# deepreinforce-ai/CUDA-L2

Measured on AMD Instinct MI355X. Metric: HGEMM TFLOP/s, higher is better.
Workload: dtype f16

## Files before the change

### cuda-l2_amd/build.py

```python
from __future__ import annotations

import concurrent.futures as cf
import hashlib
import os
import shutil
import subprocess
import sys
from pathlib import Path

PKG_DIR = Path(__file__).resolve().parent
REPO_DIR = PKG_DIR.parent
CSRC = PKG_DIR / "csrc"
INCLUDE = REPO_DIR / "include"
BUILD = PKG_DIR / "build"
OBJ = BUILD / "obj"
_SUFFIX = os.environ.get("HGEMM_LIB_SUFFIX", "")
LIB_DIR = PKG_DIR / ("lib_" + _SUFFIX if _SUFFIX else "lib")
BIN_DIR = PKG_DIR / "bin"
ROCM = Path(os.environ.get("ROCM_PATH", "/opt/rocm"))
HIPCC = str(ROCM / "bin" / "hipcc")
ARCH = "gfx950"

LIB_SOURCES = [
    "hgemm_inst_g0.hip",
    "hgemm_inst_g1.hip",
    "hgemm_inst_g2.hip",
    "hgemm_inst_g3.hip",
    "hgemm_inst_g4.hip",
    "hgemm_inst_g5.hip",
    "hgemm_inst_g6.hip",
    "hgemm_inst_g7.hip",
    "hgemm_inst_g8.hip",
    "hgemm_inst_g9.hip",
    "hgemm_inst_g10.hip",
    "hgemm_inst_g11.hip",
    "hgemm_inst_g12.hip",
    "hgemm_registry.hip",
    "hgemm_plan.hip",
    "hgemm_api.hip",
    "hgemm_baselines.hip",
]

HIP_FLAGS = os.environ.get("HGEMM_EXTRA_HIPFLAGS", "").split() + [f"--offload-arch={ARCH}", "-O3", "-std=c++17", "-fPIC", "-Wall", "-Wno-unused-function",
             "-Wno-unused-result", "-Wno-unused-value", "-DROCBLAS_NO_DEPRECATED_WARNINGS", "-D__HIP_PLATFORM_AMD__"]


def _headers_digest() -> str:
    h = hashlib.sha256()
    for d in (CSRC, INCLUDE):
        for p in sorted(d.rglob("*")):
            if p.suffix in (".hpp", ".h", ".def", ".inc"):
                h.update(p.name.encode())
                h.update(p.read_bytes())
    return h.hexdigest()


def _run(cmd: list[str], verbose: bool) -> None:
    if verbose:
        print(" ".join(cmd), flush=True)
    res = subprocess.run(cmd, capture_output=True, text=True)
    if res.returncode != 0:
        sys.stderr.write(res.stdout + res.stderr)
        raise RuntimeError(f"build step failed ({res.returncode}): {' '.join(cmd)}")
    if verbose and (res.stdout or res.stderr):
        print(res.stdout + res.stderr, flush=True)


def compile_object(src: Path, extra_flags: list[str], hdr_digest: str, verbose: bool = False) -> Path:
    OBJ.mkdir(parents=True, exist_ok=True)
    cmd_core = [HIPCC, *HIP_FLAGS, *extra_flags, f"-I{CSRC}", f"-I{INCLUDE}", "-c"]
    key = hashlib.sha256()
    key.update(" ".join(cmd_core).encode())
    key.update(hdr_digest.encode())
    key.update(src.read_bytes())
    obj = OBJ / f"{src.stem}-{key.hexdigest()[:20]}.o"
    if not obj.exists():
        tmp = obj.with_suffix(f".tmp{os.getpid()}.o")
        _run([*cmd_core, str(src), "-o", str(tmp)], verbose)
        os.replace(tmp, obj)
    return obj


def build_library(verbose: bool = False, jobs: int | None = None) -> Path:
    hdr = _headers_digest()
    jobs = jobs or min(8, os.cpu_count() or 1)
    srcs = [CSRC / s for s in LIB_SOURCES]
    with cf.ThreadPoolExecutor(max_workers=jobs) as ex:
        objs = list(ex.map(lambda s: compile_object(s, [], hdr, verbose), srcs))
    LIB_DIR.mkdir(exist_ok=True)
    lib = LIB_DIR / "libhgemm_mi355x.so"
    stamp = LIB_DIR / ".libhgemm_mi355x.stamp"
    want = hashlib.sha256(" ".join(o.name for o in objs).encode()).hexdigest()
    if lib.exists() and stamp.exists() and stamp.read_text() == want:
        return lib
    tmp = lib.with_suffix(f".tmp{os.getpid()}.so")
    _run([HIPCC, f"--offload-arch={ARCH}", "-shared", "-fPIC", *map(str, objs), "-o", str(tmp),
          f"-L{ROCM / 'lib'}", "-lrocblas", "-lhipblaslt", "-lamdhip64",
          "-Wl,--no-undefined", "-Wl,-soname,libhgemm_mi355x.so"], verbose)
    os.replace(tmp, lib)
    stamp.write_text(want)
    return lib


def build_tools(verbose: bool = False) -> list[Path]:
    lib = build_library(verbose)
    hdr = _headers_digest()
    BIN_DIR.mkdir(exist_ok=True)
    out = []
    for name in ("hgemm_tune",):
        src = CSRC / "tools" / f"{name}.cpp"
        if not src.exists():
            continue
        obj = compile_object(src, ["-x", "hip"], hdr, verbose)
        exe = BIN_DIR / name
        stamp = BIN_DIR / f".{name}.stamp"
        want = obj.name + lib.name + str(lib.stat().st_mtime_ns)
        if not (exe.exists() and stamp.exists() and stamp.read_text() == want):
            _run([HIPCC, f"--offload-arch={ARCH}", str(obj), "-o", str(exe), f"-L{LIB_DIR}", "-lhgemm_mi355x",
                  f"-L{ROCM / 'lib'}", "-lamdhip64", "-lrocm_smi64", "-Wl,-rpath,$ORIGIN/../lib", f"-Wl,-rpath,{ROCM / 'lib'}"],
# ... 61 lines not shown
```

### cuda-l2_amd/csrc/hgemm_api.hip

```cpp
#include "hgemm_plan.hpp"
#include "hgemm_kernel_nn.hpp"
#include "../../include/hgemm_mi355x.h"

#include <algorithm>
#include <atomic>
#include <cmath>
#include <cstdint>
#include <cstdlib>
#include <cstring>
#include <mutex>
#include <vector>

using namespace hgemm_mi355x;

namespace {

thread_local int g_last_hip_error = 0;
#ifdef HGEMM_ABLATION
int g_debug_flags = 0;
#endif
#ifdef HGEMM_TIMELINE
unsigned long long* g_timeline = nullptr;
int g_timeline_slots = 0;
unsigned g_timeline_count = 0;
// ... 664 lines not shown
  for (Workspace& w : g_ws)
    if (w.ptr && hipFree(w.ptr) != hipSuccess) rc = HGEMM_ERR_HIP;
  for (void* p : g_ws_retired)
    if (hipFree(p) != hipSuccess) rc = HGEMM_ERR_HIP;
  g_ws.clear();
  g_ws_retired.clear();
  return rc;
}

int hgemm_mi355x_release_stream_workspace(void* stream) {
  int dev = 0;
  if (hipGetDevice(&dev) != hipSuccess) return HGEMM_ERR_HIP;
  std::lock_guard<std::mutex> lk(g_ws_mutex);
  for (size_t i = 0; i < g_ws.size(); ++i) {
    if (g_ws[i].device != dev || g_ws[i].stream != (hipStream_t)stream) continue;
    int rc = HGEMM_OK;
    if (g_ws[i].ptr) {
      if (g_ws[i].captured) g_ws_retired.push_back(g_ws[i].ptr);
      else if (hipFree(g_ws[i].ptr) != hipSuccess) rc = HGEMM_ERR_HIP;
    }
    g_ws.erase(g_ws.begin() + (long)i);
    return rc;
  }
  return HGEMM_OK;
}

int hgemm_mi355x_reserve_workspace(int M, int N, int K, void* stream) {
  if (M <= 0 || N <= 0 || K <= 0) return HGEMM_ERR_BAD_ARG;
  int cfg = 0, splits = 1, group = 1;
  const int st = hgemm_mi355x_plan(M, N, K, &cfg, &splits, &group);
  if (st != HGEMM_OK) return st;
  const size_t ws = std::max(hgemm_mi355x_plan_workspace_bytes(cfg, splits, M, N, K), kCounterBytes + (size_t)256 * 256 * 256 * sizeof(float));
  float* slabs = nullptr; unsigned* counters = nullptr;
  const int rc = ensure_workspace(ws - kCounterBytes, (hipStream_t)stream, &slabs, &counters);
  return rc == HGEMM_ERR_NO_WORKSPACE_INTERNAL ? HGEMM_ERR_NO_WORKSPACE : rc;
}

int hgemm_mi355x_launch(int config_id, int splits_arg, int group_m, const void* a, const void* b,
                        const void* b_col_major, void* c, int M, int N, int K, int lda, int ldb,
                        int ldc, void* stream) {
  DisarmTiming disarm_timing;
  if (!a || !c || M <= 0 || N <= 0 || K <= 0) return HGEMM_ERR_BAD_ARG;
  if (config_id >= g_num_kernels || config_id < HGEMM_CONFIG_RAGGED) return HGEMM_ERR_BAD_ARG;
#ifdef HGEMM_TIMELINE
  ++g_timeline_count;
#endif
  hipStream_t s = (hipStream_t)stream;
  const bool aligned = mfma_path_ok(a, b_col_major, c, M, N, K, lda, ldb, ldc);
  unsigned ruled_out = 0;
  auto resolve = [&] {
    return resolve_launch(config_id, splits_arg, group_m, b != nullptr, b_col_major != nullptr, aligned, M, N, K, lda, ldb, ldc, ruled_out);
  };
  LaunchPlan p = resolve();
  float* slabs = nullptr; unsigned* counters = nullptr;
  while (p.status == HGEMM_OK && p.slab_bytes) {
    const int st = ensure_workspace(p.slab_bytes, s, &slabs, &counters);
    if (st == HGEMM_OK) break;
    if (st != HGEMM_ERR_NO_WORKSPACE_INTERNAL && p.form != FORM_HYBRID) return st;
    ruled_out |= 1u << p.form;
    p = resolve();
  }
  if (p.status != HGEMM_OK) return p.status;
  for (int i = 0; i < p.n; ++i) {
    GemmArgs& g = p.d[i].g;
    g.A = (const f16*)a; g.Bt = (const f16*)b_col_major; g.C = (f16*)c;
    if (p.d[i].epi != EPI_C16) {
      g.partial = slabs;
      if (p.counters) g.counters = counters;
    }
    const TimingSlot ts = timing_slot(p.d[i].start, p.d[i].stop);
    switch (p.d[i].thunk) {
      case THUNK_ENTRY: g_kernel_table[config_id].launch(g, p.d[i].grid, s, p.d[i].epi, ts); break;
      case THUNK_SPLITK_REDUCE: launch_splitk_reduce(g.partial, g.C, M, N, ldc, g.splits, s, ts); break;
      case THUNK_TAIL_REDUCE: launch_tail_reduce(g, g_kernel_table[config_id].bm, g_kernel_table[config_id].bn, s, ts); break;
      case THUNK_RAGGED: launch_ragged(g, s, ts); break;
      case THUNK_GENERIC: launch_generic((const f16*)a, (const f16*)b, (f16*)c, M, N, K, lda, N, ldc, s, ts); break;
    }
  }
  hipError_t err = hipGetLastError();
  if (err != hipSuccess) { g_last_hip_error = (int)err; return HGEMM_ERR_HIP; }
  return HGEMM_OK;
}

int hgemm_mi355x_set_insitu(int enable) {
  const int old = insitu_enabled() ? 1 : 0;
  g_insitu_mode.store(enable ? 1 : 0);
  if (!enable) {
    std::lock_guard<std::mutex> lk(g_insitu_mutex);
    g_insitu.clear();
    g_insitu_epoch.fetch_add(1, std::memory_order_release);
  }
  return old;
}

int hgemm_mi355x_insitu_enabled(void) { return insitu_enabled() ? 1 : 0; }

int hgemm_mi355x_insitu_candidates(int M, int N, int K, int config_id[3], int splits[3], int group_m[3]) {
  if (M <= 0 || N <= 0 || K <= 0 || !config_id || !splits || !group_m) return 0;
  PlanTriple c[3];
  const int n = insitu_candidates(M, N, K, c);
  for (int i = 0; i < n; ++i) { config_id[i] = c[i].cfg; splits[i] = c[i].splits; group_m[i] = c[i].group_m; }
  return n;
}

int hgemm_mi355x_insitu_choice(int M, int N, int K, int* config_id, int* splits, int* group_m) {
  PlanTriple p;
  int dev = 0;
  if (hipGetDevice(&dev) != hipSuccess) { (void)hipGetLastError(); dev = 0; }
  if (!config_id || !splits || !group_m || !insitu_lookup(dev, M, N, K, &p)) return 0;
  *config_id = p.cfg; *splits = p.splits; *group_m = p.group_m;
  return 1;
}

int hgemm_mi355x_fp32(const void* a, const void* b, const void* bt, void* c, int M, int N, int K,
                      void* stream) {
  return run(HGEMM_ACC_FP32, a, b, bt, c, M, N, K, stream);
}

int hgemm_mi355x_fp16(const void* a, const void* b, const void* bt, void* c, int M, int N, int K,
                      void* stream) {
  return run(HGEMM_ACC_FP16, a, b, bt, c, M, N, K, stream);
}

int hgemm_mi355x_nn_num_configs(void) { return kLayoutNN.t.count; }
const char* hgemm_mi355x_nn_config_name(int id) { return tr_config_name(kLayoutNN, id); }
int hgemm_mi355x_nn_config_by_name(const char* name) { return tr_config_by_name(kLayoutNN, name); }
int hgemm_mi355x_nn_config_info(int id, int out[8]) { return tr_config_info(kLayoutNN, id, out); }
int hgemm_mi355x_nn_plan(int M, int N, int K, int* nn_config, int* splits) { return tr_plan(kLayoutNN, M, N, K, nn_config, splits); }
int hgemm_mi355x_nn_runs(int nn_config, int M, int N, int K, int lda, int ldb, int ldc) { return tr_runs(kLayoutNN, TR_F16, kOutC16, nn_config, M, N, K, lda, ldb, ldc); }
size_t hgemm_mi355x_nn_plan_workspace_bytes(int nn_config, int splits, int M, int N, int K) {
  return tr_plan_workspace_bytes(kLayoutNN, nn_config, splits, M, N, K);
}
int hgemm_mi355x_nn_reserve_workspace(int M, int N, int K, void* stream) { return tr_reserve_workspace(kLayoutNN, M, N, K, stream); }
int hgemm_mi355x_launch_nn(int nn_config, int splits_arg, const void* a, const void* b, void* c, int M, int N, int K, int lda, int ldb,
                           int ldc, void* stream) {
  return tr_launch(kLayoutNN, TR_F16, kOutC16, nn_config, splits_arg, a, b, nullptr, c, M, N, K, lda, ldb, ldc, stream);
}
int hgemm_mi355x_nn_fp32(const void* a, const void* b, void* c, int M, int N, int K, void* stream) { return tr_run(kLayoutNN, TR_F16, kOutC16, a, b, nullptr, c, M, N, K, stream); }
int hgemm_mi355x_nn_fp16(const void* a, const void* b, void* c, int M, int N, int K, void* stream) { return tr_run(kLayoutNN, TR_F16, kOutC16, a, b, nullptr, c, M, N, K, stream); }
int hgemm_mi355x_selfcheck_launch_nn(int nn_config, int splits, int operands, int M, int N, int K, int lda, int ldb, int ldc, int ruled_out,
                                     long long out[20]) {
  return tr_selfcheck_launch(kLayoutNN, TR_F16, kOutC16, nn_config, splits, operands, M, N, K, lda, ldb, ldc, ruled_out, out);
}

int hgemm_mi355x_ta_num_configs(void) { return kLayoutTA.t.count; }
const char* hgemm_mi355x_ta_config_name(int id) { return tr_config_name(kLayoutTA, id); }
int hgemm_mi355x_ta_config_by_name(const char* name) { return tr_config_by_name(kLayoutTA, name); }
int hgemm_mi355x_ta_config_info(int id, int out[8]) { return tr_config_info(kLayoutTA, id, out); }
int hgemm_mi355x_ta_plan(int M, int N, int K, int* ta_config, int* splits) { return tr_plan(kLayoutTA, M, N, K, ta_config, splits); }
int hgemm_mi355x_ta_runs(int ta_config, int M, int N, int K, int lda, int ldb, int ldc) { return tr_runs(kLayoutTA, TR_F16, kOutC16, ta_config, M, N, K, lda, ldb, ldc); }
size_t hgemm_mi355x_ta_plan_workspace_bytes(int ta_config, int splits, int M, int N, int K) {
  return tr_plan_workspace_bytes(kLayoutTA, ta_config, splits, M, N, K);
}
int hgemm_mi355x_ta_reserve_workspace(int M, int N, int K, void* stream) { return tr_reserve_workspace(kLayoutTA, M, N, K, stream); }
int hgemm_mi355x_launch_ta(int ta_config, int splits_arg, const void* a_col_major, const void* b, void* c, int M, int N, int K, int lda,
                           int ldb, int ldc, void* stream) {
  return tr_launch(kLayoutTA, TR_F16, kOutC16, ta_config, splits_arg, a_col_major, b, nullptr, c, M, N, K, lda, ldb, ldc, stream);
}
int hgemm_mi355x_ta_fp32(const void* a_col_major, const void* b, void* c, int M, int N, int K, void* stream) { return tr_run(kLayoutTA, TR_F16, kOutC16, a_col_major, b, nullptr, c, M, N, K, stream); }
int hgemm_mi355x_ta_fp16(const void* a_col_major, const void* b, void* c, int M, int N, int K, void* stream) { return tr_run(kLayoutTA, TR_F16, kOutC16, a_col_major, b, nullptr, c, M, N, K, stream); }
int hgemm_mi355x_selfcheck_launch_ta(int ta_config, int splits, int operands, int M, int N, int K, int lda, int ldb, int ldc, int ruled_out,
                                     long long out[20]) {
  return tr_selfcheck_launch(kLayoutTA, TR_F16, kOutC16, ta_config, splits, operands, M, N, K, lda, ldb, ldc, ruled_out, out);
}

int hgemm_mi355x_launch_ta_c32(int ta_config, int splits_arg, const void* a_col_major, const void* b, float* c32, int M, int N, int K, int lda,
// ... 180 lines not shown
```

### cuda-l2_amd/csrc/hgemm_launch.hpp

```cpp
#pragma once
#include "hgemm_kernel_rs.hpp"
#include "hgemm_kernel_sq.hpp"
#include "hgemm_kernel_wd.hpp"
#include "hgemm_kernel_lu.hpp"

#include <hip/hip_ext.h>

namespace hgemm_mi355x {

struct LaunchTiming { hipEvent_t start = nullptr, stop = nullptr; };
extern thread_local LaunchTiming t_launch_timing;

struct TimingSlot { hipEvent_t start = nullptr, stop = nullptr; };
inline TimingSlot timing_slot(bool first, bool last) {
  TimingSlot s;
  if (first) { s.start = t_launch_timing.start; t_launch_timing.start = nullptr; }
  if (last) { s.stop = t_launch_timing.stop; t_launch_timing.stop = nullptr; }
  return s;
}

#define HGEMM_LAUNCH(KERNEL, GRID, THREADS, STREAM, SLOT, ...)                                              \
  do {                                                                                                      \
    if ((SLOT).start || (SLOT).stop)                                                                        \
      hipExtLaunchKernelGGL(KERNEL, dim3(GRID), dim3(THREADS), 0, STREAM, (SLOT).start, (SLOT).stop, 0,     \
                            __VA_ARGS__);                                                                   \
    else                                                                                                    \
      hipLaunchKernelGGL(KERNEL, dim3(GRID), dim3(THREADS), 0, STREAM, __VA_ARGS__);                        \
  } while (0)

template <class CFG>
void launch_cfg(const GemmArgs& g, int grid, hipStream_t stream, int epi, TimingSlot ts) {
  if (epi == EPI_STREAMK) {
    if constexpr (CFG::BM * CFG::BN <= 256 * 128) HGEMM_LAUNCH((hgemm_tn_sk_kernel<CFG>), grid, CFG::THREADS, stream, ts, g);
  } else if (epi == EPI_FUSED)
    HGEMM_LAUNCH((hgemm_tn_kernel<CFG, EPI_FUSED>), grid, CFG::THREADS, stream, ts, g);
  else if (epi == EPI_SLAB)
    HGEMM_LAUNCH((hgemm_tn_kernel<CFG, EPI_SLAB>), grid, CFG::THREADS, stream, ts, g);
  else
    HGEMM_LAUNCH((hgemm_tn_kernel<CFG, EPI_C16>), grid, CFG::THREADS, stream, ts, g);
}

template <class CFG>
void launch_sp(const GemmArgs& g, int grid, hipStream_t stream, int epi, TimingSlot ts) {
  const bool wide = ((g.N & 7) == 0) && ((g.ldc & 7) == 0) && ((reinterpret_cast<uintptr_t>(g.C) & 15) == 0);
  if (epi == EPI_FUSED)
    HGEMM_LAUNCH((hgemm_tn_sp_kernel<CFG, SP_EPI_FUSED>), grid, CFG::THREADS, stream, ts, g);
  else if (epi == EPI_SLAB)
    HGEMM_LAUNCH((hgemm_tn_sp_kernel<CFG, SP_EPI_SLAB>), grid, CFG::THREADS, stream, ts, g);
  else if (wide)
    HGEMM_LAUNCH((hgemm_tn_sp_kernel<CFG, SP_EPI_WIDE>), grid, CFG::THREADS, stream, ts, g);
  else
    HGEMM_LAUNCH((hgemm_tn_sp_kernel<CFG, SP_EPI_NARROW>), grid, CFG::THREADS, stream, ts, g);
}

template <class CFG, int FLAG>
void launch_sq_variant(const GemmArgs& g, int grid, hipStream_t stream, int epi, TimingSlot ts) {
  const bool wide = ((g.N & 7) == 0) && ((g.ldc & 7) == 0) && ((reinterpret_cast<uintptr_t>(g.C) & 15) == 0);
  if (epi == EPI_FUSED)
    HGEMM_LAUNCH((hgemm_tn_sq_kernel<CFG, SP_EPI_FUSED | FLAG>), grid, CFG::THREADS, stream, ts, g);
  else if (epi == EPI_SLAB)
    HGEMM_LAUNCH((hgemm_tn_sq_kernel<CFG, SP_EPI_SLAB | FLAG>), grid, CFG::THREADS, stream, ts, g);
  else if (wide)
    HGEMM_LAUNCH((hgemm_tn_sq_kernel<CFG, SP_EPI_WIDE | FLAG>), grid, CFG::THREADS, stream, ts, g);
  else
    HGEMM_LAUNCH((hgemm_tn_sq_kernel<CFG, SP_EPI_NARROW | FLAG>), grid, CFG::THREADS, stream, ts, g);
}

template <class CFG>
void launch_sq(const GemmArgs& g, int grid, hipStream_t stream, int epi, TimingSlot ts) {
  if constexpr (CFG::MI == 16) {
    if (g.K % (BK * CFG::KT) != 0) return launch_sq_variant<CFG, EPI_KTAIL>(g, grid, stream, epi, ts);
    if (g.flags & ARG_XCD_STAGGER) return launch_sq_variant<CFG, EPI_KSTAGGER>(g, grid, stream, epi, ts);
  }
  launch_sq_variant<CFG, 0>(g, grid, stream, epi, ts);
}

template <class CFG, int FLAG>
void launch_rs_variant(const GemmArgs& g, int grid, hipStream_t stream, int epi, TimingSlot ts) {
  if (epi == EPI_FUSED)
    HGEMM_LAUNCH((hgemm_tn_rs_kernel<CFG, EPI_FUSED | FLAG>), grid, CFG::THREADS, stream, ts, g);
  else if (epi == EPI_SLAB)
    HGEMM_LAUNCH((hgemm_tn_rs_kernel<CFG, EPI_SLAB | FLAG>), grid, CFG::THREADS, stream, ts, g);
  else
    HGEMM_LAUNCH((hgemm_tn_rs_kernel<CFG, EPI_C16 | FLAG>), grid, CFG::THREADS, stream, ts, g);
}

template <class CFG>
void launch_rs(const GemmArgs& g, int grid, hipStream_t stream, int epi, TimingSlot ts) {
  if (epi == EPI_STREAMK)
    HGEMM_LAUNCH((hgemm_tn_rs_sk_kernel<CFG>), grid, CFG::THREADS, stream, ts, g);
  else if (g.K % CFG::BKS != 0)
    launch_rs_variant<CFG, EPI_KTAIL>(g, grid, stream, epi, ts);
  else
    launch_rs_variant<CFG, 0>(g, grid, stream, epi, ts);
}

template <class CFG>
void launch_wd(const GemmArgs& g, int grid, hipStream_t stream, int epi, TimingSlot ts) {
  if (epi == EPI_FUSED)
    HGEMM_LAUNCH((hgemm_tn_wd_kernel<CFG, EPI_FUSED>), grid, CFG::THREADS, stream, ts, g);
  else if (epi == EPI_SLAB)
    HGEMM_LAUNCH((hgemm_tn_wd_kernel<CFG, EPI_SLAB>), grid, CFG::THREADS, stream, ts, g);
  else
    HGEMM_LAUNCH((hgemm_tn_wd_kernel<CFG, EPI_C16>), grid, CFG::THREADS, stream, ts, g);
}

template <class CFG>
void launch_lu(const GemmArgs& g, int grid, hipStream_t stream, int epi, TimingSlot ts) {
  if (epi == EPI_SLAB)
    HGEMM_LAUNCH((hgemm_tn_lu_kernel<CFG, EPI_SLAB>), grid, CFG::THREADS, stream, ts, g);
  else
    HGEMM_LAUNCH((hgemm_tn_lu_kernel<CFG, EPI_C16>), grid, CFG::THREADS, stream, ts, g);
}

enum class Family : char { T = 't', S = 's', Q = 'q', R = 'r', W = 'w', U = 'u' };
enum class KTail : char { NONE, PADDED, DIRECT };

struct KernelEntry {
  const char* name;
  Family family;
  int bm, bn, wm, wn, mi, nbuf;
  int threads, lds_bytes;
  void (*launch)(const GemmArgs&, int, hipStream_t, int, TimingSlot);
  int persistent_wgs;
  bool has_fused;
  int kgran;
  KTail ktail;
  int sk_wgs_per_cu;
  bool explicit_only;
};
inline bool w_splits_k(const KernelEntry& e) { return e.family == Family::W && e.wm * e.wn == 1; }

extern const KernelEntry g_kernel_table[];
extern const int g_num_kernels;

void launch_splitk_reduce(const float* partial, f16* C, int M, int N, int ldc, int splits,
                          hipStream_t stream, TimingSlot ts);
void launch_tail_reduce(const GemmArgs& g, int BM, int BN, hipStream_t stream, TimingSlot ts);
void launch_ragged(const GemmArgs& g, hipStream_t stream, TimingSlot ts);
void launch_generic(const f16* A, const f16* B, f16* C, int M, int N, int K, int lda, int ldb,
                    int ldc, hipStream_t stream, TimingSlot ts);

}
```

### include/hgemm_mi355x.h

```cpp
#ifndef HGEMM_MI355X_H_
#define HGEMM_MI355X_H_

#include <stddef.h>

#ifdef __cplusplus
extern "C" {
#endif

typedef enum {
  HGEMM_OK = 0,
  HGEMM_ERR_BAD_ARG = -1,
  HGEMM_ERR_TOO_LARGE = -2,
  HGEMM_ERR_HIP = -3,
  HGEMM_ERR_BACKEND = -4,
  HGEMM_ERR_NOT_READY = -5,
  HGEMM_ERR_NO_ALGO = -6,
  HGEMM_ERR_NO_WORKSPACE = -7
} hgemm_status_t;

typedef enum { HGEMM_ACC_FP32 = 0, HGEMM_ACC_FP16 = 1 } hgemm_acc_t;

#define HGEMM_CONFIG_GENERIC (-1)
#define HGEMM_CONFIG_RAGGED  (-2)

// ... 65 lines not shown
int hgemm_mi355x_launch_ta(int ta_config, int splits, const void* a_col_major, const void* b, void* c,
                           int M, int N, int K, int lda, int ldb, int ldc, void* stream);
int hgemm_mi355x_ta_num_configs(void);
const char* hgemm_mi355x_ta_config_name(int ta_config);
int hgemm_mi355x_ta_config_by_name(const char* name);
int hgemm_mi355x_ta_config_info(int ta_config, int out[8]);
int hgemm_mi355x_ta_plan(int M, int N, int K, int* ta_config, int* splits);
int hgemm_mi355x_ta_runs(int ta_config, int M, int N, int K, int lda, int ldb, int ldc);
size_t hgemm_mi355x_ta_plan_workspace_bytes(int ta_config, int splits, int M, int N, int K);
int hgemm_mi355x_ta_reserve_workspace(int M, int N, int K, void* stream);
int hgemm_mi355x_ta_c32(const void* a_col_major, const void* b, float* c32, int M, int N, int K, int accumulate, void* stream);
int hgemm_mi355x_launch_ta_c32(int ta_config, int splits, const void* a_col_major, const void* b, float* c32,
                               int M, int N, int K, int lda, int ldb, int ldc, int accumulate, void* stream);
int hgemm_mi355x_ta_c32_runs(int ta_config, int M, int N, int K, int lda, int ldb, int ldc);

int bgemm_mi355x_nn(const void* a, const void* b, void* c, int M, int N, int K, void* stream);
int bgemm_mi355x_ta(const void* a_col_major, const void* b, void* c, int M, int N, int K, void* stream);
int bgemm_mi355x_ta_c32(const void* a_col_major, const void* b, float* c32, int M, int N, int K, int accumulate, void* stream);
int bgemm_mi355x_launch_nn(int nn_config, int splits, const void* a, const void* b, void* c,
                           int M, int N, int K, int lda, int ldb, int ldc, void* stream);
int bgemm_mi355x_launch_ta(int ta_config, int splits, const void* a_col_major, const void* b, void* c,
                           int M, int N, int K, int lda, int ldb, int ldc, void* stream);
int bgemm_mi355x_launch_ta_c32(int ta_config, int splits, const void* a_col_major, const void* b, float* c32,
                               int M, int N, int K, int lda, int ldb, int ldc, int accumulate, void* stream);
int bgemm_mi355x_nn_runs(int nn_config, int M, int N, int K, int lda, int ldb, int ldc);
int bgemm_mi355x_ta_runs(int ta_config, int M, int N, int K, int lda, int ldb, int ldc);
int bgemm_mi355x_ta_c32_runs(int ta_config, int M, int N, int K, int lda, int ldb, int ldc);

int bgemm_mi355x_tn(const void* a, const void* b_col_major, void* c, int M, int N, int K, void* stream);
int bgemm_mi355x_launch_tn(int tn_config, int splits, const void* a, const void* b_col_major, void* c,
                           int M, int N, int K, int lda, int ldb, int ldc, void* stream);
int bgemm_mi355x_tn_runs(int tn_config, int M, int N, int K, int lda, int ldb, int ldc);
int bgemm_mi355x_tn_num_configs(void);
const char* bgemm_mi355x_tn_config_name(int tn_config);
int bgemm_mi355x_tn_config_by_name(const char* name);
int bgemm_mi355x_tn_config_info(int tn_config, int out[8]);
int bgemm_mi355x_tn_plan(int M, int N, int K, int* tn_config, int* splits);
size_t bgemm_mi355x_tn_plan_workspace_bytes(int tn_config, int splits, int M, int N, int K);
int bgemm_mi355x_tn_reserve_workspace(int M, int N, int K, void* stream);

int bgemm_mi355x_tn_bias(const void* a, const void* b_col_major, const void* bias, void* c, int M, int N, int K, void* stream);
int bgemm_mi355x_launch_tn_bias(int tn_config, int splits, const void* a, const void* b_col_major, const void* bias, void* c,
                                int M, int N, int K, int lda, int ldb, int ldc, void* stream);
int bgemm_mi355x_tn_bias_runs(int tn_config, int M, int N, int K, int lda, int ldb, int ldc);

const char* hgemm_mi355x_strerror(int status);
int hgemm_mi355x_last_hip_error(void);
const char* hgemm_mi355x_version(void);

int hgemm_rocblas_init(void);
int hgemm_rocblas_destroy(void);
int hgemm_rocblas_nn(const void* a, const void* b, void* c, int M, int N, int K, int acc, void* stream);
int hgemm_rocblas_tn(const void* a, const void* b_col_major, void* c, int M, int N, int K, int acc, void* stream);
int hgemm_rocblas_ta(const void* a_col_major, const void* b, void* c, int M, int N, int K, int acc, void* stream);
int bgemm_rocblas_nn(const void* a, const void* b, void* c, int M, int N, int K, void* stream);
int bgemm_rocblas_ta(const void* a_col_major, const void* b, void* c, int M, int N, int K, void* stream);
int bgemm_rocblas_tn(const void* a, const void* b_col_major, void* c, int M, int N, int K, void* stream);

int hgemm_hipblaslt_heuristic_init(void);
int hgemm_hipblaslt_heuristic_destroy(void);
int hgemm_hipblaslt_heuristic_nn(const void* a, const void* b, void* c, int M, int N, int K, int acc, void* stream);
int hgemm_hipblaslt_heuristic_tn(const void* a, const void* b_col_major, void* c, int M, int N, int K, int acc, void* stream);

int hgemm_hipblaslt_autotune_init(void);
int hgemm_hipblaslt_autotune_destroy(void);
int hgemm_hipblaslt_autotune_find_best_nn(int M, int N, int K, int acc);
int hgemm_hipblaslt_autotune_find_best_tn(int M, int N, int K, int acc);
int hgemm_hipblaslt_autotune_nn(const void* a, const void* b, void* c, int M, int N, int K, int acc, void* stream);
int hgemm_hipblaslt_autotune_tn(const void* a, const void* b_col_major, void* c, int M, int N, int K, int acc, void* stream);
int hgemm_hipblaslt_autotune_set_cache(const char* path);
int hgemm_hipblaslt_autotune_from_cache(int tn);
int hgemm_hipblaslt_autotune_cache_stats(int* hits, int* misses);
int hgemm_hipblaslt_autotune_candidates(int tn);
double hgemm_hipblaslt_autotune_best_ms(int tn);
int hgemm_hipblaslt_compute16_fallback(int which, int tn);

int hgemm_fill_normal_f16(void* device_ptr, size_t n, unsigned long long seed, void* stream);

void* hgemm_mi355x_event_create(void);
int hgemm_mi355x_event_destroy(void* event);
int hgemm_mi355x_time_next_launch(void* start_event, void* stop_event);
double hgemm_mi355x_event_elapsed_us(void* start_event, void* stop_event);

#ifdef __cplusplus
}
#endif
#endif
```

Measured before the change: 1428.

## Add specialized one-item-per-workgroup 256x256 square kernel path

Result: faster. 1449, median of 6 (+1.5%).

```diff
diff --git a/cuda-l2_amd/build.py b/cuda-l2_amd/build.py
--- a/cuda-l2_amd/build.py
+++ b/cuda-l2_amd/build.py
@@ -35,6 +35,7 @@
     "hgemm_inst_g10.hip",
     "hgemm_inst_g11.hip",
     "hgemm_inst_g12.hip",
+    "hgemm_inst_g13.hip",
     "hgemm_registry.hip",
     "hgemm_plan.hip",
     "hgemm_api.hip",
diff --git a/cuda-l2_amd/csrc/hgemm_api.hip b/cuda-l2_amd/csrc/hgemm_api.hip
--- a/cuda-l2_amd/csrc/hgemm_api.hip
+++ b/cuda-l2_amd/csrc/hgemm_api.hip
@@ -770,6 +770,21 @@
   return HGEMM_OK;
 }
 
+int hgemm_mi355x_set_one_item_kernel(int on) { return sq_one_set_enabled(on); }
+
+unsigned long long hgemm_mi355x_one_item_kernel_launches(void) { return sq_one_launch_count(); }
+
+int hgemm_mi355x_one_item_kernel_takes(int config_id, int splits, int group_m, int M, int N, int K, int lda, int ldb, int ldc) {
+  if (M <= 0 || N <= 0 || K <= 0 || config_id >= g_num_kernels || config_id < HGEMM_CONFIG_RAGGED) return HGEMM_ERR_BAD_ARG;
+  const LaunchPlan p = resolve_launch(config_id, splits, group_m, false, true, true, M, N, K, lda, ldb, ldc, 0);
+  if (p.status != HGEMM_OK) return p.status;
+  static const int q256 = hgemm_mi355x_config_by_name("q256x256_w2x2");
+  if (config_id != q256) return 0;
+  for (int i = 0; i < p.n; ++i)
+    if (p.d[i].thunk == THUNK_ENTRY && sq_one_takes(p.d[i].g, p.d[i].grid, p.d[i].epi)) return 1;
+  return 0;
+}
+
 int hgemm_mi355x_set_insitu(int enable) {
   const int old = insitu_enabled() ? 1 : 0;
   g_insitu_mode.store(enable ? 1 : 0);
diff --git a/cuda-l2_amd/csrc/hgemm_inst_g13.hip b/cuda-l2_amd/csrc/hgemm_inst_g13.hip
--- /dev/null
+++ b/cuda-l2_amd/csrc/hgemm_inst_g13.hip
@@ -0,0 +1,42 @@
+#include "hgemm_launch.hpp"
+#include "hgemm_kernel_sq_one.hpp"
+
+#include <atomic>
+
+namespace hgemm_mi355x {
+
+template __global__ void hgemm_tn_sq_one_kernel<CfgSQOne>(const GemmArgs);
+
+namespace {
+#ifdef HGEMM_TIMELINE
+std::atomic<int> g_sq_one_on{0};
+#else
+std::atomic<int> g_sq_one_on{1};
+#endif
+std::atomic<unsigned long long> g_sq_one_launches{0};
+}
+
+int sq_one_set_enabled(int on) { return g_sq_one_on.exchange(on ? 1 : 0); }
+unsigned long long sq_one_launch_count() { return g_sq_one_launches.load(); }
+
+bool sq_one_takes(const GemmArgs& g, int grid, int epi) {
+  if (!g_sq_one_on.load(std::memory_order_relaxed)) return false;
+  const bool wide = ((g.N & 7) == 0) && ((g.ldc & 7) == 0) && ((reinterpret_cast<uintptr_t>(g.C) & 15) == 0);
+  if (epi != EPI_C16 || !wide) return false;
+  if (g.K % (BK * CfgSQOne::KT) != 0 || g.K / BK < SQ_ONE_MIN_STEPS) return false;
+  if (g.splits != 1 || g.tail_tiles != 0 || g.items > grid) return false;
+  if (g.flags & (ARG_XCD_STAGGER | ARG_PHASE_OFFSET | ARG_PHASE_OFFSET4)) return false;
+#ifdef HGEMM_ABLATION
+  if (g.debug) return false;
+#endif
+  return true;
+}
+
+bool launch_sq_one(const GemmArgs& g, int grid, hipStream_t stream, int epi, TimingSlot ts) {
+  if (!sq_one_takes(g, grid, epi)) return false;
+  g_sq_one_launches.fetch_add(1, std::memory_order_relaxed);
+  HGEMM_LAUNCH((hgemm_tn_sq_one_kernel<CfgSQOne>), grid, CfgSQOne::THREADS, stream, ts, g);
+  return true;
+}
+
+}
diff --git a/cuda-l2_amd/csrc/hgemm_kernel_sq_one.hpp b/cuda-l2_amd/csrc/hgemm_kernel_sq_one.hpp
--- /dev/null
+++ b/cuda-l2_amd/csrc/hgemm_kernel_sq_one.hpp
@@ -0,0 +1,221 @@
+#pragma once
+
+#include "hgemm_kernel_sq.hpp"
+
+namespace hgemm_mi355x {
+
+using CfgSQOne = CfgSQ<256, 256, 2, 2, 1, 16>;
+constexpr int SQ_ONE_MIN_STEPS = 3;
+
+#if defined(__HIP_DEVICE_COMPILE__)
+template <class CFG, int PHASE, bool LATE, bool EARLY, int VMW, bool NEXT>
+__device__ __forceinline__ void sq1_interval(const f16x8 (&af)[CFG::NFA], const f16x8 (&bf)[CFG::NFB],
+                                             f16x8 (&lead)[PHASE == 0 ? CFG::NFB : CFG::NFA], const char* lead0, const char* lead1,
+                                             f16x8 (&trail)[PHASE == 0 ? CFG::NFA : CFG::NFB], const char* trail0, const char* trail1,
+                                             int wave, const uint32_t (&voffA)[CFG::PA], const uint32_t (&voffB)[CFG::PB],
+                                             __amdgpu_buffer_rsrc_t rs_l, char* stage_l, uint32_t kbyte_l,
+                                             __amdgpu_buffer_rsrc_t rs_e, char* stage_e, uint32_t kbyte_e) {
+  constexpr int FM = CFG::FM, FN = CFG::FN, T = CFG::T, RS = CFG::RS;
+  constexpr int NLEAD = PHASE == 0 ? CFG::NFB : CFG::NFA, FLEAD = PHASE == 0 ? FN : FM, FTRAIL = PHASE == 0 ? FM : FN;
+  constexpr int OP_E = PHASE == 0 ? 1 : 0, OP_L = PHASE == 0 ? 0 : 1;
+  constexpr int D_L = PHASE == 0 ? CFG::DA : CFG::DB;
+  constexpr int S = PHASE == 0 ? CFG::P : CFG::Q;
+  constexpr bool LEAD = PHASE == 0 || NEXT;
+  const uint32_t lds_l = (uint32_t)(uintptr_t)(lds_void_t*)stage_l + (uint32_t)wave * 1024u;
+  const uint32_t lds_e = (uint32_t)(uintptr_t)(lds_void_t*)stage_e + (uint32_t)wave * 1024u;
+#pragma unroll
+  for (int n = 0; n < T; ++n) {
+    const int u = n / (FM * FN), i = (n / FN) % FM, j = n % FN;
+    if (NEXT && n == S) {
+      __builtin_amdgcn_sched_barrier(0);
+      __builtin_amdgcn_s_waitcnt(kWaitLgkm0);
+      sp_sync();
+    }
+    sp_mfma_mi<CFG::MI>(i * FN + j, bf[u * FN + j], af[u * FM + i]);
+    if (LEAD && n % RS == 0 && n / RS < NLEAD) {
+      const int r = n / RS;
+      lead[r] = *(const f16x8*)((r / FLEAD ? lead1 : lead0) + (r % FLEAD) * CFG::MI * ROW_BYTES);
+    }
+    constexpr SqSlots<CFG, PHASE> tab{};
+    const int l = LATE ? tab.late[n] : -1, l1 = LATE ? tab.late[n + 1] : -1;
+    const int e = EARLY ? tab.early[n] : -1, e1 = EARLY ? tab.early[n + 1] : -1;
+    const int r = NEXT ? tab.trail[n] : -1;
+    if (l >= 0) { if constexpr (OP_L == 0) sq_piece_load<CFG, 0>(rs_l, voffA, D_L + l, kbyte_l); else sq_piece_load<CFG, 1>(rs_l, voffB, D_L + l, kbyte_l); }
+    if (e >= 0) { if constexpr (OP_E == 0) sq_piece_load<CFG, 0>(rs_e, voffA, e, kbyte_e); else sq_piece_load<CFG, 1>(rs_e, voffB, e, kbyte_e); }
+    if (r >= 0) trail[r] = *(const f16x8*)((r / FTRAIL ? trail1 : trail0) + (r % FTRAIL) * CFG::MI * ROW_BYTES);
+    if (l1 >= 0) sq_piece_m0<CFG, OP_L>(lds_l, D_L + l1, l1 > 0);
+    if (e1 >= 0) sq_piece_m0<CFG, OP_E>(lds_e, e1, e1 > 0);
+    if constexpr (VMW >= 0) { if (NEXT && n == S - 2) wait_vmcnt<VMW>(); }
+    if (n == T - 3) {
+      __builtin_amdgcn_sched_barrier(0);
+      __builtin_amdgcn_s_waitcnt(kWaitLgkm0);
+      __builtin_amdgcn_sched_barrier(0);
+    }
+  }
+}
+#endif
+
+#define SQ1_FRAG(STAGE, OPOFF, H) ((STAGE) + (OPOFF) + foff[H])
+#define SQ1_K_STEP(YS, ZS, LA, EB, LB, EA, VMP, VMQ, NEXT)                                                              \
+  do {                                                                                                                  \
+    char* st  = smem + (step & 1) * CFG::STAGE_BYTES;                                                                   \
+    char* nst = smem + ((step + 1) & 1) * CFG::STAGE_BYTES;                                                             \
+    sq1_interval<CFG, 0, LA, EB, VMP, NEXT>(fX, fU, fV, SQ1_FRAG(st, b_base_off, 1), SQ1_FRAG(st, b_base_off, 1),       \
+                                            ZS, SQ1_FRAG(nst, a_base_off, 1), SQ1_FRAG(nst, a_base_off, 1), wave, voffA, voffB, \
+                                            rsA, st, kbA, rsB, st, kbB);                                                \
+    kbA += ROW_BYTES;                                                                                                   \
+    sq1_interval<CFG, 1, LB, EA, VMQ, NEXT>(YS, fV, fX, SQ1_FRAG(nst, a_base_off, 0), SQ1_FRAG(nst, a_base_off, 0),     \
+                                            fU, SQ1_FRAG(nst, b_base_off, 0), SQ1_FRAG(nst, b_base_off, 0), wave, voffA, voffB, \
+                                            rsB, st, kbB, rsA, nst, kbA);                                               \
+    kbB += ROW_BYTES;                                                                                                   \
+    ++step;                                                                                                             \
+  } while (0)
+#define SQ1_FULL_STEP(YS, ZS) SQ1_K_STEP(YS, ZS, true, true, true, true, CFG::NJA + CFG::NJB, CFG::NJA + CFG::NJB, true)
+
+template <class CFG>
+__global__ void __launch_bounds__(CFG::THREADS) hgemm_tn_sq_one_kernel(const GemmArgs g) {
+  prefetch_kernargs<sizeof(GemmArgs)>();
+#if defined(__HIP_DEVICE_COMPILE__)
+  static_assert(CFG::MI == 16 && CFG::KT == 1 && CFG::WGS == 1, "the 16x16x32, K = 64 per stage, one-workgroup-per-CU member");
+  static_assert(sp_staged_ok<CFG>(CFG::LDS_BYTES), "the LDS-staged wide epilogue");
+  constexpr int BM = CFG::BM, BN = CFG::BN, FM = CFG::FM, FN = CFG::FN, MI = CFG::MI;
+  constexpr int NFA = CFG::NFA, NFB = CFG::NFB;
+#ifdef HGEMM_TIMELINE
+  constexpr int TL_EXTRA = 64;
+#else
+  constexpr int TL_EXTRA = 0;
+#endif
+  constexpr int STAGED_BYTES = CFG::NW * SP_STAGED_BYTES_PER_WAVE;
+  __shared__ __attribute__((aligned(1024))) char smem[CFG::LDS_BYTES + 64 + STAGED_BYTES + TL_EXTRA];
+
+  const int tid  = threadIdx.x;
+  HGEMM_TL_STAMP(smem + CFG::LDS_BYTES, 0, tid);
+  HGEMM_TL_REALTIME(smem + CFG::LDS_BYTES, 1, tid);
+  const int lane = tid & 63;
+  const int wave = __builtin_amdgcn_readfirstlane(tid >> 6);
+  const int wave_m = wave / CFG::WN;
+  const int wave_n = wave % CFG::WN;
+
+  const ItemWalk walk = persistent_walk(g.items);
+  if (walk.count == 0) return;
+  const TileCoord tc = map_logical(g, walk.base + walk.first, BM, BN);
+  const int m0 = __builtin_amdgcn_readfirstlane(tc.m0), n0 = __builtin_amdgcn_readfirstlane(tc.n0);
+  const int nk = __builtin_amdgcn_readfirstlane(tc.nk);
+
+  const int lr = lane & (MI - 1), lq = lane / MI, sw = (lr >> 1) & 7;
+  int foff[2];
+#pragma unroll
+  for (int h = 0; h < 2; ++h) foff[h] = lr * ROW_BYTES + (((h * 4 + lq) ^ sw) << 4);
+  const int a_base_off = wave_m * CFG::TM * ROW_BYTES;
+  const int b_base_off = BM * ROW_BYTES + wave_n * CFG::TN * ROW_BYTES;
+
+  sp_reserve_agprs<CFG::AGPRS>();
+
+  static_assert(CFG::NW % 2 == 0, "the swizzle key of a wave's row blocks must not depend on the piece");
+  const uint32_t chunk0 = (uint32_t)((lane & 7) ^ (((wave & 1) << 2) | (lane >> 4)));
+  uint32_t voffA[CFG::PA], voffB[CFG::PB];
+#pragma unroll
+  for (int q = 0; q < CFG::PA; ++q) voffA[q] = ((uint32_t)((wave + q * CFG::NW) * 8 + (lane >> 3)) * (uint32_t)g.lda + chunk0 * 8u) * 2u;
+#pragma unroll
+  for (int q = 0; q < CFG::PB; ++q) voffB[q] = ((uint32_t)((wave + q * CFG::NW) * 8 + (lane >> 3)) * (uint32_t)g.ldb + chunk0 * 8u) * 2u;
+  auto tile_rsrc = [](const f16* base, int row0, int rows, int ld) __attribute__((always_inline)) {
+    const uintptr_t addr = reinterpret_cast<uintptr_t>(base + (size_t)row0 * ld);
+    const uintptr_t uni = ((uintptr_t)(uint32_t)__builtin_amdgcn_readfirstlane((int)(addr >> 32)) << 32) |
+                          (uint32_t)__builtin_amdgcn_readfirstlane((int)(uint32_t)addr);
+    const unsigned long long rem = (unsigned long long)(rows - row0) * (unsigned long long)ld * 2ull;
+    const unsigned range = (unsigned)__builtin_amdgcn_readfirstlane((int)(rem > 0xFFFFFFFFull ? 0xFFFFFFFFu : (unsigned)rem));
+    return __builtin_amdgcn_make_buffer_rsrc((void*)uni, 0, (int)range, 0x00020000);
+  };
+  const __amdgpu_buffer_rsrc_t rsA = tile_rsrc(g.A, m0, g.M, g.lda), rsB = tile_rsrc(g.Bt, n0, g.N, g.ldb);
+  const uint32_t kb0 = (uint32_t)__builtin_amdgcn_readfirstlane(tc.k_begin * 2);
+  HGEMM_TL_STAMP(smem + CFG::LDS_BYTES + 64 + STAGED_BYTES, 0, tid);
+  constexpr int NZ = FM * FN, NPIECE = 2 * (CFG::NJA + CFG::NJB);
+  int zi = 0, pi = 0;
+#pragma unroll
+  for (int s = 0; s < 2; ++s) {
+#pragma unroll
+    for (int p = 0; p < CFG::NJA; ++p) {
+      sq_issue_piece<CFG, 0>(rsA, voffA, smem + s * CFG::STAGE_BYTES, wave, p, kb0 + s * ROW_BYTES);
+      for (++pi; zi < (pi * NZ) / NPIECE; ++zi) sp_zero_acc(zi);
+    }
+#pragma unroll
+    for (int p = 0; p < CFG::NJB; ++p) {
+      sq_issue_piece<CFG, 1>(rsB, voffB, smem + s * CFG::STAGE_BYTES, wave, p, kb0 + s * ROW_BYTES);
+      for (++pi; zi < (pi * NZ) / NPIECE; ++zi) sp_zero_acc(zi);
+    }
+  }
+  __builtin_amdgcn_sched_barrier(0);
+#pragma unroll
+  for (; zi < NZ; ++zi) sp_zero_acc(zi);
+  HGEMM_TL_STAMP(smem + CFG::LDS_BYTES + 64 + STAGED_BYTES, 1, tid);
+  wait_vmcnt<CFG::NJA + CFG::NJB>();
+  __builtin_amdgcn_s_barrier();
+  HGEMM_TL_STAMP(smem + CFG::LDS_BYTES + 64 + STAGED_BYTES, 2, tid);
+
+  f16x8 fX[NFA], fY[NFA], fZ[NFA], fU[NFB], fV[NFB];
+#pragma unroll
+  for (int r = 0; r < NFA; ++r) {
+    fX[r] = *(const f16x8*)(SQ1_FRAG(smem, a_base_off, 0) + r * MI * ROW_BYTES);
+    fY[r] = *(const f16x8*)(SQ1_FRAG(smem, a_base_off, 1) + r * MI * ROW_BYTES);
+  }
+#pragma unroll
+  for (int r = 0; r < NFB; ++r) fU[r] = *(const f16x8*)(SQ1_FRAG(smem, b_base_off, 0) + r * MI * ROW_BYTES);
+  uint32_t kbA = kb0 + 2 * ROW_BYTES, kbB = kb0 + 2 * ROW_BYTES;
+  __builtin_amdgcn_sched_barrier(0);
+  __builtin_amdgcn_s_waitcnt(kWaitLgkm0);
+  sp_sync();
+#pragma unroll
+  for (int p = 0; p < CFG::DA; ++p) sq_issue_piece<CFG, 0>(rsA, voffA, smem, wave, p, kbA);
+
+  int step = 0;
+  HGEMM_TL_STAMP(smem + CFG::LDS_BYTES, 2, tid);
+  HGEMM_TL_STAMP(smem + CFG::LDS_BYTES, 3, tid);
+  if ((nk & 1) == 0) {
+    sq_settle(fX, fY, fU);
+    SQ1_FULL_STEP(fY, fZ);
+#pragma unroll
+    for (int r = 0; r < NFA; ++r) fY[r] = fZ[r];
+  }
+  sq_settle(fX, fY, fU);
+#pragma clang loop unroll(disable)
+  for (int t = step; t + 4 < nk; t += 2) {
+    SQ1_FULL_STEP(fY, fZ);
+    SQ1_FULL_STEP(fZ, fY);
+  }
+  sq_settle(fX, fY, fU);
+  SQ1_K_STEP(fY, fZ, true, true, true, false, CFG::NJA + CFG::NJB, CFG::NJA + CFG::NJB, true);
+  SQ1_K_STEP(fZ, fY, false, false, false, false, CFG::NJB, 0, true);
+  SQ1_K_STEP(fY, fZ, false, false, false, false, -1, -1, false);
+
+  HGEMM_TL_STAMP(smem + CFG::LDS_BYTES, 4, tid);
+  sp_mfma_drain();
+  const int m_wave = m0 + wave_m * CFG::TM, n_wave = n0 + wave_n * CFG::TN;
+  __builtin_amdgcn_sched_barrier(0);
+  sp_epilogue_staged<CFG>(g, m_wave, n_wave, false, smem + CFG::LDS_BYTES + 64 + wave * SP_STAGED_BYTES_PER_WAVE);
+  __builtin_amdgcn_sched_barrier(0);
+#ifdef HGEMM_TIMELINE
+  HGEMM_TL_STAMP(smem + CFG::LDS_BYTES, 5, tid);
+  wait_vmcnt<0>();
+  HGEMM_TL_STAMP(smem + CFG::LDS_BYTES, 6, tid);
+  HGEMM_TL_REALTIME(smem + CFG::LDS_BYTES, 7, tid);
+  if (g.timeline != nullptr && tid == 0) {
+    unsigned long long* tl = g.timeline + (size_t)blockIdx.x * HGEMM_TL_WORDS;
+    unsigned hw = 0, xcc = 0;
+    asm volatile("s_getreg_b32 %0, hwreg(HW_REG_HW_ID)\n\ts_getreg_b32 %1, hwreg(HW_REG_XCC_ID)" : "=s"(hw), "=s"(xcc));
+#pragma unroll
+    for (int w = 0; w < 8; ++w) tl[w] = hgemm_tl_get(smem + CFG::LDS_BYTES, w);
+#pragma unroll
+    for (int w = 0; w < 3; ++w) tl[11 + w] = hgemm_tl_get(smem + CFG::LDS_BYTES + 64 + STAGED_BYTES, w);
+    tl[8] = ((unsigned long long)xcc << 32) | hw; tl[9] = (unsigned long long)step; tl[10] = 1ull;
+  }
+#endif
+#endif
+}
+
+#undef SQ1_FULL_STEP
+#undef SQ1_K_STEP
+#undef SQ1_FRAG
+
+extern template __global__ void hgemm_tn_sq_one_kernel<CfgSQOne>(const GemmArgs);
+
+}
diff --git a/cuda-l2_amd/csrc/hgemm_launch.hpp b/cuda-l2_amd/csrc/hgemm_launch.hpp
--- a/cuda-l2_amd/csrc/hgemm_launch.hpp
+++ b/cuda-l2_amd/csrc/hgemm_launch.hpp
@@ -5,6 +5,8 @@
 #include "hgemm_kernel_lu.hpp"
 
 #include <hip/hip_ext.h>
+
+#include <type_traits>
 
 namespace hgemm_mi355x {
 
@@ -66,8 +68,16 @@
     HGEMM_LAUNCH((hgemm_tn_sq_kernel<CFG, SP_EPI_NARROW | FLAG>), grid, CFG::THREADS, stream, ts, g);
 }
 
+bool launch_sq_one(const GemmArgs& g, int grid, hipStream_t stream, int epi, TimingSlot ts);
+bool sq_one_takes(const GemmArgs& g, int grid, int epi);
+int sq_one_set_enabled(int on);
+unsigned long long sq_one_launch_count();
+
 template <class CFG>
 void launch_sq(const GemmArgs& g, int grid, hipStream_t stream, int epi, TimingSlot ts) {
+  if constexpr (std::is_same_v<CFG, CfgSQ<256, 256, 2, 2, 1, 16>>) {
+    if (launch_sq_one(g, grid, stream, epi, ts)) return;
+  }
   if constexpr (CFG::MI == 16) {
     if (g.K % (BK * CFG::KT) != 0) return launch_sq_variant<CFG, EPI_KTAIL>(g, grid, stream, epi, ts);
     if (g.flags & ARG_XCD_STAGGER) return launch_sq_variant<CFG, EPI_KSTAGGER>(g, grid, stream, epi, ts);
diff --git a/include/hgemm_mi355x.h b/include/hgemm_mi355x.h
--- a/include/hgemm_mi355x.h
+++ b/include/hgemm_mi355x.h
@@ -171,6 +171,10 @@
 int hgemm_mi355x_time_next_launch(void* start_event, void* stop_event);
 double hgemm_mi355x_event_elapsed_us(void* start_event, void* stop_event);
 
+int hgemm_mi355x_set_one_item_kernel(int on);
+unsigned long long hgemm_mi355x_one_item_kernel_launches(void);
+int hgemm_mi355x_one_item_kernel_takes(int config_id, int splits, int group_m, int M, int N, int K, int lda, int ldb, int ldc);
+
 #ifdef __cplusplus
 }
 #endif
```
